# victordeleau/MUI-DeepAutoEncoder

Hardware: AMD Instinct MI355X
Metric: training samples/sec at 3x512-dim input, batch 8192 (higher is better)
Workload: dtype bf16; 1 GPU; embedding.yaml topology: 3 slots x 512 (io 1536), z=io, 4+4 layers -> 10 x Linear(1536,1536); batch 8192 rows per GPU, Adam lr 1e-5 wd 1e-4 clip 1.0, slot-blanking k=1; global_batch=8192, parallelism=dp1

## Files before the change

### include/codae_hip.h

```cpp
#ifndef CODAE_HIP_H
#define CODAE_HIP_H

#include <stddef.h>
#include <stdint.h>

#ifdef __cplusplus
extern "C" {
#endif

#define CODAE_ABI_VERSION 11

enum {
    CODAE_OK = 0,
    CODAE_E_INVALID = -1,
    CODAE_E_HIP = -2,
    CODAE_E_UNSUPPORTED = -3
};

enum {
    CODAE_PREC_F32 = 0,
    CODAE_PREC_BF16 = 1
};

enum {
// ... 181 lines not shown
int codae_side_stream(codae_handle h, void** stream_out);
int codae_join(codae_handle h, void* stream);

int codae_span_sumsq(const float* g, int64_t n, double* acc, void* stream);
int codae_step_update_span(codae_handle h, const codae_buffers* bufs, const codae_hyper* hyper, int64_t lo, int64_t hi,
                           const double* total_sq, void* stream);
int codae_sync_transposed(codae_handle h, const codae_buffers* bufs, void* stream);
int codae_train_step(codae_handle h, const codae_buffers* bufs, const codae_batch* batch,
                     const codae_hyper* hyper, void* stream);
int codae_dp_unique_id(void* out, int32_t capacity);
int codae_dp_init(codae_handle h, const void* unique_id, int32_t rank, int32_t world);
int codae_dp_destroy(codae_handle h);
int codae_train_step_dp(codae_handle h, const codae_buffers* bufs, const codae_batch* batch, const codae_hyper* hyper,
                        int32_t n_buckets, const int32_t* bucket_lo, const int32_t* bucket_hi, void* stream);
int codae_step_path(codae_handle h, const codae_buffers* bufs, int32_t B);
int codae_set_input_noise(codae_handle h, const codae_noise* noise);
int codae_set_loss_emphasis(codae_handle h, const codae_emphasis* emphasis);
int codae_set_recon_loss(codae_handle h, const codae_recon_loss* loss);
int codae_set_hidden_dropout(codae_handle h, const codae_dropout* d);
int codae_set_slot_contrast(codae_handle h, const codae_slot_contrast* contrast);
int codae_set_optimizer(codae_handle h, const codae_optimizer* opt);
int codae_set_slot_presence(codae_handle h, const uint8_t* present, int64_t n_rows, int32_t n_slots);
int codae_set_dataset_image(codae_handle h, const float* data, const void* image_bf16, int64_t n_rows, int32_t io);
int codae_set_tied_weights(codae_handle h, int32_t on);
int codae_graph_captures(codae_handle h);
int codae_eval_step(codae_handle h, const codae_buffers* bufs, const codae_batch* batch, float* out_y,
                    void* stream);

enum {
    CODAE_K_GEMM_FWD = 0,
    CODAE_K_GEMM_DGRAD = 1,
    CODAE_K_GEMM_WGRAD = 2,
    CODAE_K_LOSS = 3,
    CODAE_K_GATHER = 4,
    CODAE_K_SUMSQ = 5,
    CODAE_K_ADAM = 6,
    CODAE_K_SLAB_REDUCE = 7,
    CODAE_K_CHAIN = 8,
    CODAE_K_BIAS_FINISH = 9,
    CODAE_K_DROPOUT = 10,
    CODAE_K_COUNT = 11
};
int codae_profile_begin(codae_handle h, uint32_t class_mask, int32_t max_records);
int codae_profile_stride(codae_handle h, int32_t every_n_steps);
int codae_profile_end(codae_handle h, int32_t* kinds, float* ms, int32_t capacity, int32_t* n_out);

// ... 118 lines not shown
```

### mui-deepautoencoder_amd/codae/hip/__init__.py

```python
import ctypes as C
import os

_HERE = os.path.dirname(os.path.abspath(__file__))
LIB_PATH = os.environ.get("CODAE_HIP_LIB") or os.path.join(_HERE, "libcodae_hip.so")

PREC_F32 = 0
PREC_BF16 = 1

ABI_VERSION = 11
S_SQ_FULL, S_SQ_PARTIAL, S_GRAD_SQ, S_LAST_LOSS, S_STEP_SQ, S_CLIP_COEF = 0, 1, 2, 3, 4, 5
S_GRAD_SQ_SLOTS, S_N_SLOTS, S_ADAM_STEP, S_COUNT = 8, 64, 72, 80
ACT_NONE, ACT_RELU, ACT_LEAKY, ACT_RELU6, ACT_ELU, ACT_SOFTPLUS, ACT_HARDSIGMOID = 0, 1, 2, 3, 4, 5, 6
NOISE_NONE, NOISE_GAUSSIAN, NOISE_MASKING, NOISE_SALT_PEPPER = 0, 1, 2, 3
LOSS_MSE, LOSS_L1, LOSS_SMOOTH_L1, LOSS_HUBER, LOSS_SLOT_COSINE = 0, 1, 2, 3, 4
OPT_ADAM, OPT_ADAMW, OPT_SGD = 0, 1, 2
SCHED_CONSTANT, SCHED_COSINE, SCHED_LINEAR, SCHED_STEP = 0, 1, 2, 3
KERNEL_CLASSES = ("gemm_fwd", "gemm_dgrad", "gemm_wgrad", "loss", "gather", "sumsq", "adam", "slab_reduce", "chain",
                  "bias_finish", "dropout")


class HipError(RuntimeError):
    pass


# ... 84 lines not shown
    "codae_step_update": (C.c_int, [_P, C.POINTER(Buffers), C.POINTER(Hyper), _P]),
    "codae_step_backward_async": (C.c_int, [_P, C.POINTER(Buffers), _I32, _I32, _I32, _P]),
    "codae_side_stream": (C.c_int, [_P, C.POINTER(C.c_void_p)]),
    "codae_profile_stride": (C.c_int, [_P, _I32]),
    "codae_join": (C.c_int, [_P, _P]),
    "codae_span_sumsq": (C.c_int, [_P, _I64, _P, _P]),
    "codae_step_update_span": (C.c_int, [_P, C.POINTER(Buffers), C.POINTER(Hyper), _I64, _I64, _P, _P]),
    "codae_sync_transposed": (C.c_int, [_P, C.POINTER(Buffers), _P]),
    "codae_train_step": (C.c_int, [_P, C.POINTER(Buffers), C.POINTER(Batch), C.POINTER(Hyper), _P]),
    "codae_train_step_graph": (C.c_int, [_P, C.POINTER(Buffers), C.POINTER(Batch), C.POINTER(Hyper), _P]),
    "codae_set_input_noise": (C.c_int, [_P, C.POINTER(Noise)]),
    "codae_set_loss_emphasis": (C.c_int, [_P, C.POINTER(Emphasis)]),
    "codae_set_recon_loss": (C.c_int, [_P, C.POINTER(ReconLoss)]),
    "codae_set_hidden_dropout": (C.c_int, [_P, C.POINTER(Dropout)]),
    "codae_set_slot_contrast": (C.c_int, [_P, C.POINTER(SlotContrast)]),
    "codae_set_optimizer": (C.c_int, [_P, C.POINTER(Optimizer)]),
    "codae_optimizer_update": (C.c_int, [_P, _P, _P, _P, _P, _I64, C.POINTER(Hyper), C.POINTER(Optimizer), _P, _P]),
    "codae_graph_captures": (C.c_int, [_P]),
    "codae_set_tied_weights": (C.c_int, [_P, _I32]),
    "codae_tie_fold": (C.c_int, [_P, C.POINTER(TiePair), _I32, _P]),
    "codae_tie_mirror": (C.c_int, [_P, _P, _P, C.POINTER(TiePair), _I32, _P]),
    "codae_set_slot_presence": (C.c_int, [_P, _P, _I64, _I32]),
    "codae_set_dataset_image": (C.c_int, [_P, _P, _P, _I64, _I32]),
    "codae_corrupt_batch_present": (C.c_int, [C.POINTER(Batch), C.POINTER(Noise), _I32, _P, _P, _I32, _I64, _P, _I32, _P]),
    "codae_mse_loss_present": (C.c_int, [C.POINTER(Batch), _P, _P, _I32, _I64, _F, _P, _P, _P, _I32, _P]),
    "codae_emph_loss_present": (C.c_int, [C.POINTER(Batch), C.POINTER(Noise), _I32, C.POINTER(Emphasis), _P, _P, _I32, _I64, _F, _P, _P,
                                          _P, _I32, _P]),
    "codae_recon_loss_fwd_bwd_present": (C.c_int, [C.POINTER(Batch), C.POINTER(Noise), _I32, C.POINTER(Emphasis), C.POINTER(ReconLoss), _P,
                                                   _P, _I32, _I64, _F, _P, _P, _P, _I32, _P]),
    "codae_slot_contrast_prepare_present": (C.c_int, [_P, _I32, C.POINTER(SlotContrast), _I32, _I32, _P, _I32, _P]),
    "codae_slot_contrast_fwd_bwd_present": (C.c_int, [C.POINTER(Batch), C.POINTER(Noise), _I32, C.POINTER(Emphasis),
                                                      C.POINTER(SlotContrast), _P, _P, _I32, _I64, _F, _P, _P, _P, _I32, _P]),
    "codae_slot_contrast_ws_bytes": (_I64, [_I32, _I32, _I32, _I32]),
    "codae_slot_contrast_prepare": (C.c_int, [_P, _I32, C.POINTER(SlotContrast), _I32, _I32, _P]),
    "codae_slot_contrast_fwd_bwd": (C.c_int, [C.POINTER(Batch), C.POINTER(Noise), _I32, C.POINTER(Emphasis), C.POINTER(SlotContrast), _P, _P,
                                              _I32, _I64, _F, _P, _P, _P]),
    "codae_slot_contrast_blocks": (C.c_int, [_I32]),
    "codae_dropout_fwd": (C.c_int, [_P, _I32, _I64, _I32, _I32, _P, _I32, _I32, _F, C.c_uint64, _P]),
    "codae_dropout_bwd": (C.c_int, [_P, _I32, _I64, _I32, _I32, _P, _I32, _I32, _F, C.c_uint64, _P, _P]),
    "codae_dropout_blocks": (C.c_int, [_I32]),
    "codae_emph_loss": (C.c_int, [C.POINTER(Batch), C.POINTER(Noise), _I32, C.POINTER(Emphasis), _P, _P, _I32, _I64, _F, _P, _P, _P]),
    "codae_emph_loss_blocks": (C.c_int, [_I32]),
    "codae_recon_loss_fwd_bwd": (C.c_int, [C.POINTER(Batch), C.POINTER(Noise), _I32, C.POINTER(Emphasis), C.POINTER(ReconLoss), _P, _P, _I32, _I64,
                                           _F, _P, _P, _P]),
    "codae_recon_loss_blocks": (C.c_int, [_I32]),
    "codae_corrupt_batch": (C.c_int, [C.POINTER(Batch), C.POINTER(Noise), _I32, _P, _P, _I32, _I64, _P]),
# ... 100 lines not shown
```

### mui-deepautoencoder_amd/codae/hip/engine.py

```python
import ctypes as C

import torch

from . import (PREC_BF16, PREC_F32, S_COUNT, S_GRAD_SQ, S_GRAD_SQ_SLOTS, S_LAST_LOSS, S_N_SLOTS, S_SQ_FULL, S_SQ_PARTIAL,
               Batch, Buffers, Dropout, Emphasis,
               HipError, Hyper, Sizes, Spec, TiePair, check, current_stream, lib, ptr)


def precision_code(precision):
    if precision in (PREC_F32, "f32", "fp32", "parity"):
        return PREC_F32
    if precision in (PREC_BF16, "bf16", "throughput"):
        return PREC_BF16
    raise ValueError("unknown precision %r (use 'f32' or 'bf16')" % (precision,))


def _tie_pair_array(pairs):
    arr = (TiePair * max(len(pairs), 1))()
    for i, (e, d, r, c) in enumerate(pairs):
        arr[i] = TiePair(int(e), int(d), int(r), int(c))
    return arr


def tie_fold(grads, pairs):
# ... 59 lines not shown
            if int(sz.n_scalars) != S_COUNT:
                raise HipError("library reports %d scalars, binding expects %d" % (int(sz.n_scalars), S_COUNT))
            self.scalars = torch.zeros(int(sz.n_scalars), dtype=torch.float64, device=device)
        self.bufs = Buffers(ptr(self._params), ptr(self.grads), ptr(self.adam_m), ptr(self.adam_v), ptr(self.shadow),
                            ptr(self.acts), ptr(self.dacts), ptr(self.slabs), ptr(self.scalars), ptr(self.shadow_t),
                            ptr(self.bias_parts))
        self.w_off, self.b_off = [], []
        for l in range(self.L):
            w, b, s = C.c_int64(), C.c_int64(), C.c_int64()
            check(self._lib.codae_param_offsets(self._h, l, C.byref(w), C.byref(b), C.byref(s)))
            self.w_off.append(w.value)
            self.b_off.append(b.value)
        self.input_noise = None
        self.loss_emphasis = None
        self._emph_weights = None
        self.hidden_dropout = None
        self.recon_loss = None
        self.slot_contrast = None
        self._contrast_pins = None
        self.slot_presence = None
        self._presence_table = None
        self.tied_weights = False
        self._dataset_image = None
        self.optimizer = None
        self.adam_vmax = None
        self.step_count = 0
        self.generation = 0

    def _layer_acts(self, activation):
        if activation is None:
            return None
        if isinstance(activation, (list, tuple)) and len(activation) == self.L and all(
                isinstance(a, (list, tuple)) for a in activation):
            acts = [tuple(a) for a in activation]
        else:
            if isinstance(activation, (list, tuple)):
                one = tuple(activation)
            else:
                from ..model.activation import from_factory
                one = from_factory(activation)
            acts = [one if s[2] else (0, 0.0, 0.0, 0.0) for s in self.schedule]
        for a in acts:
            if len(a) != 4:
                raise HipError("activation per layer must be (kind, p0, p1, p2), got %r" % (a,))
        return [(int(a[0]), float(a[1]), float(a[2]), float(a[3])) for a in acts]

# ... 62 lines not shown
            check(self._lib.codae_backward(self._h, C.byref(self.bufs), ptr(dy), ptr(dx), dy.shape[0], layer_lo,
                                           layer_hi, current_stream()))
        return dx

    def make_batch(self, data, row_idx, mask_id, mask_table, B=None, mask_to_use=None, run=0):
        if data.dtype != torch.float32 or not data.is_contiguous() or data.device != self.device:
            raise HipError("batch data must be a contiguous fp32 tensor on %s" % self.device)
        for name, t in (("row_idx", row_idx), ("mask_id", mask_id)):
            if t is not None and (t.dtype != torch.int32 or t.device != self.device or not t.is_contiguous()):
                raise HipError("%s must be a contiguous int32 tensor on %s" % (name, self.device))
        if mask_table is not None and (mask_table.dtype != torch.uint8 or mask_table.device != self.device):
            raise HipError("mask_table must be a uint8 tensor on %s" % self.device)
        if B is None:
            B = int(row_idx.numel()) if row_idx is not None else int(data.shape[0])
        nb_run = 0
        if mask_to_use is not None:
            if mask_to_use.dtype != torch.int32 or mask_to_use.device != self.device or not mask_to_use.is_contiguous() \
                    or mask_to_use.dim() != 2 or mask_to_use.shape[0] != data.shape[0]:
                raise HipError("mask_to_use must be a contiguous int32 [n_rows, nb_run] tensor on %s" % self.device)
            nb_run = int(mask_to_use.shape[1])
        b = Batch(ptr(data), ptr(row_idx), ptr(mask_id), ptr(mask_table), int(B), int(data.shape[1]),
                  ptr(mask_to_use), nb_run, int(run))
        b._pinned = (data, row_idx, mask_id, mask_table, mask_to_use)
        return b

    def hyper(self, lr, weight_decay, clip=1.0, global_rows=0, betas=(0.9, 0.999), eps=1e-8, step=None):
        return Hyper(lr, weight_decay, betas[0], betas[1], eps, clip if clip else 0.0,
                     self.step_count + 1 if step is None else step, float(global_rows))

    def set_input_noise(self, noise):
        if noise is not None and not hasattr(noise, "as_struct"):
            raise HipError("set_input_noise: expected a codae.tool.InputNoise or None, got %r" % (noise,))
        st = None if noise is None else noise.as_struct()
        check(self._lib.codae_set_input_noise(self._h, None if st is None else C.byref(st)))
        self.input_noise = noise

    def set_loss_emphasis(self, emphasis, n_slots=None):
        if emphasis is not None and not hasattr(emphasis, "column_weights"):
            raise HipError("set_loss_emphasis: expected a codae.tool.LossEmphasis or None, got %r" % (emphasis,))
        weights = None
        if emphasis is not None:
            cw = emphasis.column_weights(self.schedule[-1][1], n_slots)
            if cw is not None:
                weights = torch.from_numpy(cw).to(self.device).contiguous()
        self._set_emphasis_struct(None if emphasis is None else Emphasis(emphasis.alpha, emphasis.beta, ptr(weights)))
        self._emph_weights = weights
# ... 235 lines not shown
```

### mui-deepautoencoder_amd/csrc/codae_common.h

```cpp
#pragma once
#include <hip/hip_runtime.h>
#include <stdint.h>
#include <stdio.h>
#include <type_traits>

#include "codae_hip.h"

namespace codae {

void set_error(const char* fmt, ...);

#define CODAE_HIP_CHECK(expr)                                                              \
    do {                                                                                   \
        hipError_t e_ = (expr);                                                            \
        if (e_ != hipSuccess) {                                                            \
            codae::set_error("%s failed: %s (%s:%d)", #expr, hipGetErrorString(e_), __FILE__, __LINE__); \
            return CODAE_E_HIP;                                                            \
        }                                                                                  \
    } while (0)

#define CODAE_LAUNCH_CHECK()                                                               \
    do {                                                                                   \
        hipError_t e_ = hipGetLastError();                                                 \
        if (e_ != hipSuccess) {                                                            \
// ... 169 lines not shown
    __device__ __forceinline__ void store16(void* p, uint32_t byte_off, u32x4 v) const {
        if constexpr (POL == STORE_PLAIN) *reinterpret_cast<u32x4*>(p) = v;
        else __builtin_amdgcn_raw_buffer_store_b128(v, rsrc, (int)byte_off, 0, 16);
    }
};

struct EnvToggles {
    int gemm_tile = -1;
    int gemm_dbg = 0;
    int wgrad_splitk = 0;
    int small_tile_max = 200;
    int small_stages = 4;
    int f32_gemm = 0;
    int group_tile = -1;
    bool side_priority_set = false; int side_priority = 0;
    bool no_wt = false, single_stream = false, tail_on_side = false, no_fused_loss = false, flat_adam = false,
         no_fused_norm = false, no_chain = false, no_deep_small = false,
         no_relu_bits = false,
         no_prefetch = false,
         no_defer_wgrad = false;
    bool no_folded_loss_finish = false;
    bool no_folded_bias_finish = false;
    bool no_dataset_image = false;
    int store_policy = -1;
};
const EnvToggles& env();
void env_reload();

struct GemmF32 {
    const float* A; int64_t a_rs, a_ks;
    const float* B; int64_t b_rs, b_ks;
    float* C; int64_t ldc;
    int M, N, K;
    const float* bias;
    int relu;
    const float* relu_src;
    int64_t ld_relu;
    float* colsum_part;
    const int* m_dev;
    int split_k;
    int act;
    float act_p[3];
};
int gemm_f32(const GemmF32& g, hipStream_t s);
int gemm_f32x3(const GemmF32& g, hipStream_t s);
bool gemm_f32x3_takes(const GemmF32& g);
// ... 1 lines not shown

constexpr int CODAE_GROUP_MAX = 16;
struct GemmF32Group {
    int n;
    GemmF32 g[CODAE_GROUP_MAX];
    int wg_begin[CODAE_GROUP_MAX + 1];
};
int gemm_f32x3_grouped(GemmF32Group& grp, hipStream_t s);

enum { OP_KC = 0,
       OP_KS = 1
};
struct LossFuse {
    int enabled;
    const float* data;
    const int32_t* row_idx;
    const int32_t* mask_id;
    const int32_t* mask_to_use;
    int nb_run, run;
    const uint8_t* table;
    int io;
    int B;
    float inv_n;
    double* parts;
};

struct GemmBf16 {
    const bf16_t* A; int64_t lda; int a_mode;
    const bf16_t* B; int64_t ldb; int b_mode;
    void* C; int64_t ldc; int c_f32;
    int M, N, K;
    const float* bias;
    int relu;
    const bf16_t* relu_src; int64_t ld_relu;
    float* colsum_part;
    int split_k;
    LossFuse loss;
    int dbg;
    uint8_t* relu_bits_out; const uint8_t* relu_bits; int64_t ld_bits;
    const void* prefetch; int64_t prefetch_bytes;
    int coscheduled;
    double* sumsq_slots;
    int act;
    float act_p[3];
    int store_policy;
};
// ... 156 lines not shown
```

### mui-deepautoencoder_amd/csrc/engine.hip

```cpp
#include <stdarg.h>
#include <stdlib.h>
#include <string.h>

#include <cmath>
#include <vector>

#include "layer_gemm.h"
#include <dlfcn.h>
#include <rccl/rccl.h>

namespace codae {

static thread_local char g_err[512] = "";

void set_error(const char* fmt, ...) {
    va_list ap;
    va_start(ap, fmt);
    vsnprintf(g_err, sizeof(g_err), fmt, ap);
    va_end(ap);
}

static EnvToggles g_env;
static bool g_env_loaded = false;

void env_reload() {
    EnvToggles e;
    if (const char* t = getenv("CODAE_GEMM_TILE")) {
        switch (t[0]) { case 's': e.gemm_tile = 0; break; case 'q': e.gemm_tile = 3; break; case 'x': e.gemm_tile = 6; break; case 'm': e.gemm_tile = 7; break; default: break; }
    }
    if (const char* d = getenv("CODAE_GEMM_DBG")) e.gemm_dbg = atoi(d);
    if (const char* k = getenv("CODAE_WGRAD_SPLITK")) e.wgrad_splitk = atoi(k) > 0 ? atoi(k) : 0;
    if (const char* k = getenv("CODAE_GROUP_TILE")) e.group_tile = (k[0] >= '0' && k[0] <= '2') ? k[0] - '0' : -1;
    if (const char* pr = getenv("CODAE_SIDE_PRIORITY")) { e.side_priority_set = true; e.side_priority = atoi(pr); }
    e.no_wt = getenv("CODAE_NO_WT") != nullptr;
    e.single_stream = getenv("CODAE_SINGLE_STREAM") != nullptr;
    e.tail_on_side = getenv("CODAE_TAIL_ON_SIDE") != nullptr;
    e.no_fused_loss = getenv("CODAE_NO_FUSED_LOSS") != nullptr;
    e.flat_adam = getenv("CODAE_FLAT_ADAM") != nullptr;
    e.no_fused_norm = getenv("CODAE_NO_FUSED_NORM") != nullptr;
    e.no_chain = getenv("CODAE_NO_CHAIN") != nullptr;
    e.no_deep_small = getenv("CODAE_NO_DEEP_SMALL") != nullptr;
    e.no_defer_wgrad = getenv("CODAE_NO_DEFER_WGRAD") != nullptr;
    e.no_prefetch = getenv("CODAE_NO_PREFETCH") != nullptr;
    e.no_relu_bits = getenv("CODAE_NO_RELU_BITS") != nullptr;
    e.no_folded_loss_finish = getenv("CODAE_NO_FOLDED_LOSS_FINISH") != nullptr;
    e.no_dataset_image = getenv("CODAE_NO_DATASET_IMAGE") != nullptr;
    e.no_folded_bias_finish = getenv("CODAE_NO_FOLDED_BIAS_FINISH") != nullptr;
    if (const char* k = getenv("CODAE_STORE_POLICY"))
        e.store_policy = !strcmp(k, "plain") ? STORE_PLAIN : (!strcmp(k, "wt") ? STORE_WT : -1);
    if (const char* k = getenv("CODAE_F32_GEMM")) e.f32_gemm = k[0] == 'n' ? 1 : (k[0] == 'x' ? 2 : 0);
    if (const char* k = getenv("CODAE_SMALL_TILE_MAX")) e.small_tile_max = atoi(k);
    if (const char* k = getenv("CODAE_SMALL_STAGES")) e.small_stages = atoi(k) == 2 ? 2 : 4;
    g_env = e;
    g_env_loaded = true;
}

const EnvToggles& env() {
    if (!g_env_loaded) env_reload();
    return g_env;
}

}

using namespace codae;

constexpr int CODAE_MAX_DACT = 16;

struct codae_engine {
    int L = 0;
    std::vector<int> in, out;
    std::vector<int> in_ld, out_ld;
    std::vector<uint8_t> relu;
    std::vector<uint8_t> act;
    std::vector<float> act_p;
    int max_batch = 0, max_rows = 0;
    int prec = CODAE_PREC_F32;
    std::vector<int64_t> w_off, b_off;
    int64_t n_param = 0, bias_begin = 0;
    int maxw = 0;
    std::vector<int64_t> act_off;
    int64_t act_bytes = 0, dact_one = 0, slab_bytes = 0;
    std::vector<int64_t> bits_off;
    int n_dact = 3;
    std::vector<int> split_k;
    std::vector<int64_t> part_off;
    int64_t part_floats = 0;
    int64_t loss_part_off = 0;
    int loss_part_cap = 0;
    bool chain_ok = false;
    struct PresCfg { const uint8_t* table; int64_t n_rows; int32_t n_slots; int32_t reserved; };
    struct DropCfg { float p[64]; uint64_t seed; int32_t on; int32_t reserved; };
    struct ImageCfg { const float* data; const void* image; int64_t n_rows; int32_t io; int32_t reserved; };
    struct TrainCfg {
        codae_noise noise;
        codae_emphasis emph;
        int32_t emph_on, reserved;
        codae_recon_loss recon;
        codae_slot_contrast contrast;
        PresCfg pres;
        DropCfg drop;
        codae_optimizer opt;
        int32_t tied, tied_reserved;
        ImageCfg img;
    } tc;
    bool recon_on() const { return tc.recon.kind != CODAE_LOSS_MSE; }
    bool contrast_on() const { return tc.contrast.weight != 0.f; }
    int n_free() const { return (L + 1) / 2; }
    std::vector<codae_tie_pair> tie_pairs;
    bool plain_mse() const { return !tc.emph_on && !recon_on() && !contrast_on() && tc.pres.table == nullptr; }
    int graph_captures = 0;
    bool drop_live = false;
    int drop_B = 0;
    const int32_t* drop_rows = nullptr;
    int32_t drop_step = 0;
    std::vector<int> parts_pending;
    hipStream_t side = nullptr;
    hipEvent_t ev_ready[CODAE_MAX_DACT] = {}, ev_join = nullptr, ev_w[CODAE_MAX_DACT] = {};
    unsigned ready_turn = 0;
    bool w_pending[CODAE_MAX_DACT] = {};
    bool side_dirty = false;
    bool norm_scalars_zero = false;
    bool prof_on = false;
    uint32_t prof_mask = 0;
    int prof_n = 0;
    int prof_every = 1, prof_step = 0;
    hipGraphExec_t graph_exec = nullptr;
// ... 985 lines not shown
        if (!noised && gathers_from_image(h, batch, act_ptr(h, b, 0)))
            rc = launch_gather_image(batch, reinterpret_cast<const bf16_t*>(h->tc.img.image), reinterpret_cast<bf16_t*>(act_ptr(h, b, 0)), s,
                                     h->in_ld[0], zero_norm, pres, pres_slots);
        else
            rc = launch_gather_noise(batch, noised ? &h->tc.noise : nullptr, noised ? hyper->step : 0, step_dev(h, b),
                                     act_ptr(h, b, 0), bf, s, h->in_ld[0], nullptr, zero_norm, pres, pres_slots);
    }
    if (rc) return rc;
    rc = zero_pad_rows(h, act_ptr(h, b, 0), B, rows, h->in_ld[0], s);
    if (rc) return rc;
    float* y = out_y ? out_y : reinterpret_cast<float*>(act_ptr(h, b, L));
    GroupScope fwd_group(h, CODAE_K_GEMM_FWD, s);
    if (h->drop_live) fwd_group.close();
    for (int l = 0; l < L; ++l) {
        const bool last = (l == L - 1);
        if (last && fuse_loss) {
            fwd_group.close();
            GemmBf16 g = layer_fwd_bf16(h, b, l, act_ptr(h, b, l), dact_ptr(h, b, l), h->out_ld[l], false, rows);
            g.colsum_part = part_ptr(h, b, l);
            g.loss.enabled = 1; g.loss.data = batch->data; g.loss.row_idx = batch->row_idx; g.loss.mask_id = batch->mask_id;
            g.loss.mask_to_use = batch->mask_to_use; g.loss.nb_run = batch->nb_run; g.loss.run = batch->run;
            g.loss.table = batch->mask_table; g.loss.io = batch->io; g.loss.B = B; g.loss.inv_n = (float)loss_inv_n(hyper, batch);
            g.loss.parts = loss_parts_ptr(h, b);
            if (b->shadow_wt != nullptr && l >= 1 && !h->cfg.no_wt && !h->cfg.no_prefetch) {
                g.prefetch = reinterpret_cast<const bf16_t*>(b->shadow_wt) + h->w_off[l];
                g.prefetch_bytes = (int64_t)h->in[l] * h->out[l] * 2;
            }
            const int n_loss_parts = gemm_bf16_loss_parts(g);
            CODAE_REQUIRE(n_loss_parts <= h->loss_part_cap, "fused loss: %d workgroups exceed the partial-sum rows (%d)", n_loss_parts, h->loss_part_cap);
            {
                ProfScope prof(h, CODAE_K_LOSS, s);
                rc = gemm_bf16(g, s);
            }
            if (rc) return rc;
            h->parts_pending[l] = gemm_bf16_colsum_rows(g);
            h->norm_scalars_zero = true;
            if (fold_finish) {
                fold->scalars = b->scalars; fold->inv_n = 1.0 / ((double)B * batch->io);
                fold->parts = loss_parts_ptr(h, b); fold->n_parts = n_loss_parts;
                return CODAE_OK;
            }
            return finish_loss(h, b, batch, n_loss_parts, s);
        }
        rc = last ? run_linear(h, b, l, act_ptr(h, b, l), y, true, B, s)
                  : run_linear(h, b, l, act_ptr(h, b, l), act_ptr(h, b, l + 1), false, rows, s);
        if (rc) return rc;
// ... 92 lines not shown
        CODAE_REQUIRE(n_rows >= 1, "codae_set_slot_presence: n_rows %lld must be >= 1", (long long)n_rows);
        CODAE_REQUIRE(!(h->recon_on() && h->tc.recon.kind == CODAE_LOSS_SLOT_COSINE) || h->tc.recon.n_slots == n_slots,
                      "codae_set_slot_presence: n_slots %d differs from slot_cosine's %d", n_slots, h->tc.recon.n_slots);
        CODAE_REQUIRE(!h->contrast_on() || (h->tc.contrast.n_slots == n_slots && (int64_t)h->tc.contrast.n_rows <= n_rows),
                      "codae_set_slot_presence: %d slots / %lld rows do not fit the slot contrast (%d slots, %d rows)", n_slots,
                      (long long)n_rows, h->tc.contrast.n_slots, h->tc.contrast.n_rows);
        p.table = present; p.n_rows = n_rows; p.n_slots = n_slots;
    }
    h->tc.pres = p;
    return CODAE_OK;
}

int codae_set_dataset_image(codae_handle h, const float* data, const void* image_bf16, int64_t n_rows, int32_t io) {
    CODAE_REQUIRE(h != nullptr, "codae_set_dataset_image: null handle");
    codae_engine::ImageCfg im{};
    if (image_bf16 != nullptr) {
        CODAE_REQUIRE(data != nullptr, "codae_set_dataset_image: an image without the dataset it was cast from");
        CODAE_REQUIRE(n_rows >= 1, "codae_set_dataset_image: n_rows %lld must be >= 1", (long long)n_rows);
        CODAE_REQUIRE(io == h->in[0], "codae_set_dataset_image: io %d does not match the model (%d)", io, h->in[0]);
        CODAE_REQUIRE((reinterpret_cast<uintptr_t>(image_bf16) & 15) == 0, "codae_set_dataset_image: the image must be 16-byte aligned");
        im.data = data; im.image = image_bf16; im.n_rows = n_rows; im.io = io;
    }
    h->tc.img = im;
    return CODAE_OK;
}

int codae_set_optimizer(codae_handle h, const codae_optimizer* opt) {
    CODAE_REQUIRE(h != nullptr, "codae_set_optimizer: null handle");
    int rc = check_optimizer(opt);
    if (rc) return rc;
    h->tc.opt = optimizer_canonical(opt);
    return CODAE_OK;
}

int codae_set_tied_weights(codae_handle h, int32_t on) {
    CODAE_REQUIRE(h != nullptr, "codae_set_tied_weights: null handle");
    if (on) {
        for (int l = 0; l < h->L / 2; ++l) {
            const int m = h->L - 1 - l;
            if (h->in[l] != h->out[m] || h->out[l] != h->in[m]) {
                set_error("tied weights: layers %d and %d are not mirror images (%d -> %d against %d -> %d)", l, m, h->in[l], h->out[l],
                          h->in[m], h->out[m]);
                return CODAE_E_UNSUPPORTED;
            }
        }
        h->tie_pairs.clear();
// ... 358 lines not shown
```

### mui-deepautoencoder_amd/csrc/gemm_bf16_pipe.hip

```cpp
#include "codae_common.h"
#include <type_traits>

namespace codae {
namespace {

#include "gemm_bf16_halftile.h"

constexpr int TIMELINE_WGS = 4096, TIMELINE_SLOTS = 6;
__device__ unsigned long long g_timeline[TIMELINE_WGS * TIMELINE_SLOTS];

constexpr int PARK_BIAS_BYTES = 1024;
template <int BM, int BN, bool C_F32, int EPI>
constexpr int pipe_smem_bytes() {
    const bool park = BM == 256;
    return 2 * (BM + BN) * 128 + (EPI == 3 ? BM * 8 : 0) + (park ? PARK_BIAS_BYTES : 0) + (park && !C_F32 && (EPI == 0 || EPI == 2 || EPI == 4) ? BM * BN / 8 : 0);
}

template <int BM, int BN, int WM, int WN, int NLB, int A_MODE, int B_MODE, bool C_F32, int DBG = 0, int EPI = 0, int POL = STORE_PLAIN>
__device__ __forceinline__ void gemm_bf16_pipe_tile(const GemmBf16& g, int tiles_n, int tiles_mn, int kt_total, int wg, int nwg,
                                                    char* smem_raw) {
    constexpr int NW = WM * WN;
    constexpr int SM = BM / WM, SN = BN / WN;
    constexpr int AHR = BM / 2, BHR = BN / 2;
    constexpr int TMH = SM / 32, TNH = SN / 32;
    constexpr int AH = AHR * 128, BH = BHR * 128;
    constexpr int BUF = 2 * AH + 2 * BH;
    constexpr int NLA = (NLB == 4 && NW == 8) ? 4 : (((AHR / 8) % NW == 0) ? NW : 8);
    constexpr int NA = AHR / 8 / NLA, NB = BHR / 8 / NLB;
    static_assert(NLB <= NW && NLA <= NW && (AHR / 8) % NLA == 0 && (BHR / 8) % NLB == 0, "loader waves");
    static_assert(SM % 32 == 0 && SN % 32 == 0, "wave sub-tile must split into 16-wide half tiles");
    lds_char* smem = (lds_char*)smem_raw;
    constexpr bool PARK = BM == 256;
    constexpr bool PARK_BITS = PARK && !C_F32 && (EPI == 0 || EPI == 2 || EPI == 4);
    constexpr int BIAS_OFF = 2 * BUF + (EPI == 3 ? BM * 8 : 0), BITS_OFF = BIAS_OFF + PARK_BIAS_BYTES;
    static_assert(BN * 4 <= PARK_BIAS_BYTES && BN % 32 == 0, "bias slice: one 16-B piece per lane of one wave");

    const int lane = threadIdx.x & 63;
    const int w = __builtin_amdgcn_readfirstlane(threadIdx.x >> 6);
    const int wr = w / WN, wc = w % WN;

    int bid = wg;
    if (nwg > 0) {
        const int q = nwg >> 3, r = nwg & 7, xcd = bid & 7;
        bid = (xcd < r ? xcd * (q + 1) : r * (q + 1) + (xcd - r) * q) + (bid >> 3);
    }
    const int z = bid / tiles_mn;
    const int tmn = bid - z * tiles_mn;
    constexpr int TILE_GROUP_M = 4;
    const int tiles_m = tiles_mn / tiles_n;
    const int grp = tmn / (TILE_GROUP_M * tiles_n);
    const int tm0 = grp * TILE_GROUP_M;
    const int gsz = tiles_m - tm0 < TILE_GROUP_M ? tiles_m - tm0 : TILE_GROUP_M;
    const int within = tmn - grp * (TILE_GROUP_M * tiles_n);
    const int tn = within / gsz, tm = tm0 + (within - tn * gsz);
    const int i0 = tm * BM, j0 = tn * BN;
    const int kt_begin = (int)((int64_t)kt_total * z / g.split_k);
    const int kt_end = (int)((int64_t)kt_total * (z + 1) / g.split_k);
// ... 17 lines not shown
        }
    }
    if constexpr (EPI == 3) {
        const LossFuse& L = g.loss;
        int* rowinfo = reinterpret_cast<int*>(smem_raw + 2 * BUF);
        for (int r = threadIdx.x; r < BM; r += 64 * NW) {
            const int i = i0 + r;
            int src = -1, id = 0;
            if (i < L.B && i < g.M) {
                src = L.row_idx ? L.row_idx[i] : i;
                if (L.mask_id != nullptr) id = L.mask_id[i];
                else if (L.mask_to_use != nullptr) id = L.mask_to_use[(int64_t)src * L.nb_run + L.run];
            }
            rowinfo[2 * r] = src; rowinfo[2 * r + 1] = id;
        }
    }

    const bool has_bias = g.bias != nullptr;
    if constexpr (PARK) {
        if (has_bias && w == NW - 1) {
            int j = j0 + 4 * lane;
            j = j + 4 <= g.N ? j : g.N - 4;
            __builtin_amdgcn_global_load_lds((gvoid*)(g.bias + j), (__attribute__((address_space(3))) void*)(smem + BIAS_OFF), 16, 0, 0);
        }
    }
    if constexpr (PARK_BITS) {
        if (g.relu_bits != nullptr) {
            constexpr int DPR = BN / 32, NI = BM * DPR / 64;
            static_assert((BM * DPR) % 64 == 0, "bit tile: whole 64-lane instructions");
#pragma unroll
            for (int q0 = 0; q0 < NI; q0 += NW) {
                const int ins = q0 + w;
                if (ins < NI) {
                    const int q = ins * 64 + lane, r = q / DPR, cd = q - r * DPR;
                    const int row = i0 + r < g.M ? i0 + r : g.M - 1;
                    int off = (j0 >> 3) + 4 * cd;
                    off = off + 4 <= (int)g.ld_bits ? off : (int)g.ld_bits - 4;
                    __builtin_amdgcn_global_load_lds((gvoid*)(g.relu_bits + (int64_t)row * g.ld_bits + off),
                                                     (__attribute__((address_space(3))) void*)(smem + BITS_OFF + ins * 256), 4, 0, 0);
                }
            }
        }
    }
    auto bias4 = [&](int jl) -> float4 {
        if constexpr (PARK) {
            const f32x4 v = *reinterpret_cast<const __attribute__((address_space(3))) f32x4*>(smem + BIAS_OFF + jl * 4);
// ... 191 lines not shown
        }
        asm volatile("" ::"v"(pf_val));
    };
    phase_barrier();
    if constexpr (EPI == 3) {
        const LossFuse& L = g.loss;
        const int* rowinfo = reinterpret_cast<const int*>(smem_raw + 2 * BUF);
        const bool masked = (L.mask_id != nullptr) || (L.mask_to_use != nullptr);
        const uint8_t* tb = masked ? L.table : reinterpret_cast<const uint8_t*>(L.data);
        constexpr int NT = 64 * NW;
        constexpr int PITCH = BN * 2 + 16;
        static_assert(BM * PITCH <= 2 * BUF, "output tile must fit in the staging buffers");
        float sq = 0.f, sqp = 0.f;
        float cs[2][TNH][4];
        int jcl[2][TNH];
        bool jok[2][TNH];
#pragma unroll
        for (int nh = 0; nh < 2; ++nh)
#pragma unroll
            for (int nt = 0; nt < TNH; ++nt) {
                const int j = j0 + nh * BHR + wc * (SN / 2) + 16 * nt + g4;
                jok[nh][nt] = j < g.N;
                jcl[nh][nt] = jok[nh][nt] ? j : 0;
                const float4 bj = bias4(nh * BHR + wc * (SN / 2) + 16 * nt + g4);
#pragma unroll
                for (int mh = 0; mh < 2; ++mh)
#pragma unroll
                    for (int mt = 0; mt < TMH; ++mt) {
                        acc[mh][mt][nh][nt][0] += bj.x; acc[mh][mt][nh][nt][1] += bj.y;
                        acc[mh][mt][nh][nt][2] += bj.z; acc[mh][mt][nh][nt][3] += bj.w;
                    }
#pragma unroll
                for (int k = 0; k < 4; ++k) cs[nh][nt][k] = 0.f;
            }
        const int jbase = j0 + wc * (SN / 2) + g4;
        auto loss_rows = [&](auto full_tag) {
            constexpr bool FULL = decltype(full_tag)::value;
#pragma unroll
            for (int mh = 0; mh < 2; ++mh) {
                float4 xv[TMH][2][TNH];
                uint32_t mk[TMH][2][TNH];
                bool live[TMH];
#pragma unroll
                for (int mt = 0; mt < TMH; ++mt) {
                    const int il = mh * AHR + wr * (SM / 2) + 16 * mt + li;
                    const int src = rowinfo[2 * il], id = rowinfo[2 * il + 1];
                    live[mt] = src >= 0;
                    const float* xrow = L.data + (int64_t)(src >= 0 ? src : 0) * L.io;
                    const uint8_t* mrow = tb + (int64_t)id * L.io;
#pragma unroll
                    for (int nh = 0; nh < 2; ++nh)
#pragma unroll
                        for (int nt = 0; nt < TNH; ++nt) {
                            const int off = FULL ? jbase + (nh * BHR + 16 * nt) : jcl[nh][nt];
                            xv[mt][nh][nt] = *reinterpret_cast<const float4*>(xrow + off);
                            const uint32_t mv = *reinterpret_cast<const uint32_t*>(mrow + off);
                            mk[mt][nh][nt] = masked ? mv : 0x01010101u;
                        }
                }
#pragma unroll
                for (int mt = 0; mt < TMH; ++mt) {
                    const int il = mh * AHR + wr * (SM / 2) + 16 * mt + li;
#pragma unroll
                    for (int nh = 0; nh < 2; ++nh)
#pragma unroll
                        for (int nt = 0; nt < TNH; ++nt) {
                            const int jl = nh * BHR + wc * (SN / 2) + 16 * nt + g4;
                            const f32x4 a = acc[mh][mt][nh][nt];
                            const float4 x = xv[mt][nh][nt];
                            const float yv[4] = {a[0], a[1], a[2], a[3]};
                            const float xs[4] = {x.x, x.y, x.z, x.w};
                            const bool on = live[mt] && (FULL || jok[nh][nt]);
                            float gq[4];
#pragma unroll
                            for (int k = 0; k < 4; ++k) {
                                const float d = on ? xs[k] - yv[k] : 0.f;
                                const float se = d * d;
                                sq += se;
                                asm volatile("" : "+v"(sq));
                                sqp += ((mk[mt][nh][nt] >> (8 * k)) & 0xffu) == 0 ? se : 0.f;
                                gq[k] = on ? -2.f * d * L.inv_n : 0.f;
                                cs[nh][nt][k] += gq[k];
                            }
                            u32x2 o;
                            o[0] = pack_bf16x2(gq[0], gq[1]);
                            o[1] = pack_bf16x2(gq[2], gq[3]);
                            *reinterpret_cast<__attribute__((address_space(3))) u32x2*>(smem + il * PITCH + jl * 2) = o;
                        }
                }
                __builtin_amdgcn_sched_barrier(0);
            }
        };
        if (j0 + BN <= g.N) loss_rows(std::true_type{}); else loss_rows(std::false_type{});
        stamp(3);
        phase_barrier();
        {
            constexpr int CH = BN / 8, RL = NT / CH;
            const int c = threadIdx.x % CH, rl = threadIdx.x / CH;
            const int j = j0 + c * 8;
            bf16_t* Cb = reinterpret_cast<bf16_t*>(g.C);
            const TileStore<POL> out(Cb + (int64_t)i0 * g.ldc);
            constexpr int ITER = (BM + RL - 1) / RL;
#pragma unroll
            for (int it = 0; it < ITER; ++it) {
                const int r = rl + it * RL;
                const bool ok = rl < RL && j < g.N && r < BM && i0 + r < g.M;
                const u32x4 lv = *reinterpret_cast<const __attribute__((address_space(3))) u32x4*>(smem + (ok ? r : 0) * PITCH + c * 16);
                if (ok) out.store16(Cb + (int64_t)(i0 + r) * g.ldc + j, (uint32_t)(r * (int)g.ldc + j) * 2u, lv);
            }
        }
        if constexpr (dbg_time) { wait_vmcnt<0>(); stamp(4); }
#pragma unroll
        for (int o2 = 32; o2 > 0; o2 >>= 1) { sq += __shfl_xor(sq, o2); sqp += __shfl_xor(sqp, o2); }
#pragma unroll
        for (int nh = 0; nh < 2; ++nh)
#pragma unroll
            for (int nt = 0; nt < TNH; ++nt)
#pragma unroll
                for (int k = 0; k < 4; ++k) {
                    float v = cs[nh][nt][k];
                    v += __shfl_xor(v, 1); v += __shfl_xor(v, 2); v += __shfl_xor(v, 4); v += __shfl_xor(v, 8);
                    cs[nh][nt][k] = v;
                }
        phase_barrier();
        float* red = reinterpret_cast<float*>(smem_raw);
        static_assert((WM * BN + 2 * NW) * 4 <= 2 * BUF, "reduction scratch must fit");
        if (li == 0) {
#pragma unroll
            for (int nh = 0; nh < 2; ++nh)
#pragma unroll
                for (int nt = 0; nt < TNH; ++nt) {
                    const int jl = nh * BHR + wc * (SN / 2) + 16 * nt + g4;
#pragma unroll
// ... 454 lines not shown
```

Baseline: 7.333 million samples/s.

## Park the slot mask table in LDS and pipeline loss-epilogue row fetches

The Python engine now registers the batch mask table with the native handle. When the table has at most 16 masks, the fused loss GEMM epilogue copies each tile's mask slices into shared memory with global_load_lds instead of reading a mask row from global memory per output row. With the masks parked, the epilogue also double-buffers its work by quarters: it fetches the data rows for the next quarter while computing the current one, hiding load latency. The cost is extra LDS per block, which may lower occupancy, plus more register pressure. Partial tiles fall back to the old path.

```diff
diff --git a/include/codae_hip.h b/include/codae_hip.h
--- a/include/codae_hip.h
+++ b/include/codae_hip.h
@@ -227,6 +227,7 @@
 int codae_set_optimizer(codae_handle h, const codae_optimizer* opt);
 int codae_set_slot_presence(codae_handle h, const uint8_t* present, int64_t n_rows, int32_t n_slots);
 int codae_set_dataset_image(codae_handle h, const float* data, const void* image_bf16, int64_t n_rows, int32_t io);
+int codae_set_mask_table(codae_handle h, const uint8_t* mask_table, int32_t n_masks);
 int codae_set_tied_weights(codae_handle h, int32_t on);
 int codae_graph_captures(codae_handle h);
 int codae_eval_step(codae_handle h, const codae_buffers* bufs, const codae_batch* batch, float* out_y,
diff --git a/mui-deepautoencoder_amd/codae/hip/__init__.py b/mui-deepautoencoder_amd/codae/hip/__init__.py
--- a/mui-deepautoencoder_amd/codae/hip/__init__.py
+++ b/mui-deepautoencoder_amd/codae/hip/__init__.py
@@ -130,6 +130,7 @@
     "codae_tie_mirror": (C.c_int, [_P, _P, _P, C.POINTER(TiePair), _I32, _P]),
     "codae_set_slot_presence": (C.c_int, [_P, _P, _I64, _I32]),
     "codae_set_dataset_image": (C.c_int, [_P, _P, _P, _I64, _I32]),
+    "codae_set_mask_table": (C.c_int, [_P, _P, _I32]),
     "codae_corrupt_batch_present": (C.c_int, [C.POINTER(Batch), C.POINTER(Noise), _I32, _P, _P, _I32, _I64, _P, _I32, _P]),
     "codae_mse_loss_present": (C.c_int, [C.POINTER(Batch), _P, _P, _I32, _I64, _F, _P, _P, _P, _I32, _P]),
     "codae_emph_loss_present": (C.c_int, [C.POINTER(Batch), C.POINTER(Noise), _I32, C.POINTER(Emphasis), _P, _P, _I32, _I64, _F, _P, _P,
diff --git a/mui-deepautoencoder_amd/codae/hip/engine.py b/mui-deepautoencoder_amd/codae/hip/engine.py
--- a/mui-deepautoencoder_amd/codae/hip/engine.py
+++ b/mui-deepautoencoder_amd/codae/hip/engine.py
@@ -105,6 +105,7 @@
         self._presence_table = None
         self.tied_weights = False
         self._dataset_image = None
+        self._mask_table_known = None
         self.optimizer = None
         self.adam_vmax = None
         self.step_count = 0
@@ -213,6 +214,12 @@
         b = Batch(ptr(data), ptr(row_idx), ptr(mask_id), ptr(mask_table), int(B), int(data.shape[1]),
                   ptr(mask_to_use), nb_run, int(run))
         b._pinned = (data, row_idx, mask_id, mask_table, mask_to_use)
+        known = None
+        if mask_table is not None and mask_table.dim() == 2 and mask_table.is_contiguous() and mask_table.shape[1] == data.shape[1]:
+            known = (ptr(mask_table), int(mask_table.shape[0]))
+        if known != self._mask_table_known:
+            check(self._lib.codae_set_mask_table(self._h, *(known or (None, 0))))
+            self._mask_table_known = known
         return b
 
     def hyper(self, lr, weight_decay, clip=1.0, global_rows=0, betas=(0.9, 0.999), eps=1e-8, step=None):
diff --git a/mui-deepautoencoder_amd/csrc/codae_common.h b/mui-deepautoencoder_amd/csrc/codae_common.h
--- a/mui-deepautoencoder_amd/csrc/codae_common.h
+++ b/mui-deepautoencoder_amd/csrc/codae_common.h
@@ -215,6 +215,7 @@
     bool no_folded_loss_finish = false;
     bool no_folded_bias_finish = false;
     bool no_dataset_image = false;
+    bool no_loss_mask_park = false;
     int store_policy = -1;
 };
 const EnvToggles& env();
@@ -262,6 +263,7 @@
     int io;
     int B;
     float inv_n;
+    int n_masks;
     double* parts;
 };
 
diff --git a/mui-deepautoencoder_amd/csrc/engine.hip b/mui-deepautoencoder_amd/csrc/engine.hip
--- a/mui-deepautoencoder_amd/csrc/engine.hip
+++ b/mui-deepautoencoder_amd/csrc/engine.hip
@@ -46,6 +46,7 @@
     e.no_folded_loss_finish = getenv("CODAE_NO_FOLDED_LOSS_FINISH") != nullptr;
     e.no_dataset_image = getenv("CODAE_NO_DATASET_IMAGE") != nullptr;
     e.no_folded_bias_finish = getenv("CODAE_NO_FOLDED_BIAS_FINISH") != nullptr;
+    e.no_loss_mask_park = getenv("CODAE_NO_LOSS_MASK_PARK") != nullptr;
     if (const char* k = getenv("CODAE_STORE_POLICY"))
         e.store_policy = !strcmp(k, "plain") ? STORE_PLAIN : (!strcmp(k, "wt") ? STORE_WT : -1);
     if (const char* k = getenv("CODAE_F32_GEMM")) e.f32_gemm = k[0] == 'n' ? 1 : (k[0] == 'x' ? 2 : 0);
@@ -91,6 +92,7 @@
     struct PresCfg { const uint8_t* table; int64_t n_rows; int32_t n_slots; int32_t reserved; };
     struct DropCfg { float p[64]; uint64_t seed; int32_t on; int32_t reserved; };
     struct ImageCfg { const float* data; const void* image; int64_t n_rows; int32_t io; int32_t reserved; };
+    struct MaskCfg { const uint8_t* table; int32_t n_masks; int32_t reserved; };
     struct TrainCfg {
         codae_noise noise;
         codae_emphasis emph;
@@ -102,6 +104,7 @@
         codae_optimizer opt;
         int32_t tied, tied_reserved;
         ImageCfg img;
+        MaskCfg masks;
     } tc;
     bool recon_on() const { return tc.recon.kind != CODAE_LOSS_MSE; }
     bool contrast_on() const { return tc.contrast.weight != 0.f; }
@@ -1133,6 +1136,7 @@
             g.loss.mask_to_use = batch->mask_to_use; g.loss.nb_run = batch->nb_run; g.loss.run = batch->run;
             g.loss.table = batch->mask_table; g.loss.io = batch->io; g.loss.B = B; g.loss.inv_n = (float)loss_inv_n(hyper, batch);
             g.loss.parts = loss_parts_ptr(h, b);
+            if (!h->cfg.no_loss_mask_park && batch->mask_table != nullptr && batch->mask_table == h->tc.masks.table) g.loss.n_masks = h->tc.masks.n_masks;
             if (b->shadow_wt != nullptr && l >= 1 && !h->cfg.no_wt && !h->cfg.no_prefetch) {
                 g.prefetch = reinterpret_cast<const bf16_t*>(b->shadow_wt) + h->w_off[l];
                 g.prefetch_bytes = (int64_t)h->in[l] * h->out[l] * 2;
@@ -1271,6 +1275,17 @@
         im.data = data; im.image = image_bf16; im.n_rows = n_rows; im.io = io;
     }
     h->tc.img = im;
+    return CODAE_OK;
+}
+
+int codae_set_mask_table(codae_handle h, const uint8_t* mask_table, int32_t n_masks) {
+    CODAE_REQUIRE(h != nullptr, "codae_set_mask_table: null handle");
+    codae_engine::MaskCfg m{};
+    if (mask_table != nullptr) {
+        CODAE_REQUIRE(n_masks >= 1, "codae_set_mask_table: n_masks %d must be >= 1", n_masks);
+        m.table = mask_table; m.n_masks = n_masks;
+    }
+    h->tc.masks = m;
     return CODAE_OK;
 }
 
diff --git a/mui-deepautoencoder_amd/csrc/gemm_bf16_pipe.hip b/mui-deepautoencoder_amd/csrc/gemm_bf16_pipe.hip
--- a/mui-deepautoencoder_amd/csrc/gemm_bf16_pipe.hip
+++ b/mui-deepautoencoder_amd/csrc/gemm_bf16_pipe.hip
@@ -10,10 +10,12 @@
 __device__ unsigned long long g_timeline[TIMELINE_WGS * TIMELINE_SLOTS];
 
 constexpr int PARK_BIAS_BYTES = 1024;
+constexpr int PARK_MASKS = 16;
 template <int BM, int BN, bool C_F32, int EPI>
 constexpr int pipe_smem_bytes() {
     const bool park = BM == 256;
-    return 2 * (BM + BN) * 128 + (EPI == 3 ? BM * 8 : 0) + (park ? PARK_BIAS_BYTES : 0) + (park && !C_F32 && (EPI == 0 || EPI == 2 || EPI == 4) ? BM * BN / 8 : 0);
+    return 2 * (BM + BN) * 128 + (EPI == 3 ? BM * 8 : 0) + (park ? PARK_BIAS_BYTES : 0) + (park && EPI == 3 ? PARK_MASKS * BN : 0) +
+           (park && !C_F32 && (EPI == 0 || EPI == 2 || EPI == 4) ? BM * BN / 8 : 0);
 }
 
 template <int BM, int BN, int WM, int WN, int NLB, int A_MODE, int B_MODE, bool C_F32, int DBG = 0, int EPI = 0, int POL = STORE_PLAIN>
@@ -33,6 +35,7 @@
     constexpr bool PARK = BM == 256;
     constexpr bool PARK_BITS = PARK && !C_F32 && (EPI == 0 || EPI == 2 || EPI == 4);
     constexpr int BIAS_OFF = 2 * BUF + (EPI == 3 ? BM * 8 : 0), BITS_OFF = BIAS_OFF + PARK_BIAS_BYTES;
+    constexpr int MASK_OFF = BIAS_OFF + PARK_BIAS_BYTES;
     static_assert(BN * 4 <= PARK_BIAS_BYTES && BN % 32 == 0, "bias slice: one 16-B piece per lane of one wave");
 
     const int lane = threadIdx.x & 63;
@@ -96,6 +99,30 @@
             int j = j0 + 4 * lane;
             j = j + 4 <= g.N ? j : g.N - 4;
             __builtin_amdgcn_global_load_lds((gvoid*)(g.bias + j), (__attribute__((address_space(3))) void*)(smem + BIAS_OFF), 16, 0, 0);
+        }
+    }
+    bool mask_parked = false;
+    if constexpr (EPI == 3 && PARK) {
+        const LossFuse& L = g.loss;
+        mask_parked = (L.mask_id != nullptr || L.mask_to_use != nullptr) && L.n_masks >= 1 && L.n_masks <= PARK_MASKS;
+        if (mask_parked) {
+            constexpr int PPR = BN / 4, NI_MAX = PARK_MASKS * PPR / 64;
+            static_assert((PARK_MASKS * PPR) % 64 == 0, "mask slices: whole 64-lane instructions");
+            const int ni = (L.n_masks * PPR + 63) >> 6;
+#pragma unroll
+            for (int q0 = 0; q0 < NI_MAX; q0 += NW) {
+                const int ins = q0 + (NW - 1 - w);
+                if (ins < ni) {
+                    const int q = ins * 64 + lane;
+                    int m = q / PPR;
+                    const int cg = q - m * PPR;
+                    m = m < L.n_masks ? m : L.n_masks - 1;
+                    int j = j0 + 4 * cg;
+                    j = j + 4 <= g.N ? j : g.N - 4;
+                    __builtin_amdgcn_global_load_lds((gvoid*)(L.table + (int64_t)m * L.io + j),
+                                                     (__attribute__((address_space(3))) void*)(smem + MASK_OFF + ins * 256), 4, 0, 0);
+                }
+            }
         }
     }
     if constexpr (PARK_BITS) {
@@ -333,6 +360,12 @@
                 const int j = j0 + nh * BHR + wc * (SN / 2) + 16 * nt + g4;
                 jok[nh][nt] = j < g.N;
                 jcl[nh][nt] = jok[nh][nt] ? j : 0;
+            }
+        const int jbase = j0 + wc * (SN / 2) + g4;
+#pragma unroll
+        for (int nh = 0; nh < 2; ++nh)
+#pragma unroll
+            for (int nt = 0; nt < TNH; ++nt) {
                 const float4 bj = bias4(nh * BHR + wc * (SN / 2) + 16 * nt + g4);
 #pragma unroll
                 for (int mh = 0; mh < 2; ++mh)
@@ -344,82 +377,107 @@
 #pragma unroll
                 for (int k = 0; k < 4; ++k) cs[nh][nt][k] = 0.f;
             }
-        const int jbase = j0 + wc * (SN / 2) + g4;
-        auto loss_rows = [&](auto full_tag) {
-            constexpr bool FULL = decltype(full_tag)::value;
-#pragma unroll
-            for (int mh = 0; mh < 2; ++mh) {
-                float4 xv[TMH][2][TNH];
-                uint32_t mk[TMH][2][TNH];
-                bool live[TMH];
-#pragma unroll
-                for (int mt = 0; mt < TMH; ++mt) {
-                    const int il = mh * AHR + wr * (SM / 2) + 16 * mt + li;
-                    const int src = rowinfo[2 * il], id = rowinfo[2 * il + 1];
-                    live[mt] = src >= 0;
-                    const float* xrow = L.data + (int64_t)(src >= 0 ? src : 0) * L.io;
-                    const uint8_t* mrow = tb + (int64_t)id * L.io;
-#pragma unroll
-                    for (int nh = 0; nh < 2; ++nh)
-#pragma unroll
-                        for (int nt = 0; nt < TNH; ++nt) {
-                            const int off = FULL ? jbase + (nh * BHR + 16 * nt) : jcl[nh][nt];
-                            xv[mt][nh][nt] = *reinterpret_cast<const float4*>(xrow + off);
+        auto write_dy = [&]() {
+            stamp(3);
+            phase_barrier();
+            {
+                constexpr int CH = BN / 8, RL = NT / CH;
+                const int c = threadIdx.x % CH, rl = threadIdx.x / CH;
+                const int j = j0 + c * 8;
+                bf16_t* Cb = reinterpret_cast<bf16_t*>(g.C);
+                const TileStore<POL> out(Cb + (int64_t)i0 * g.ldc);
+                constexpr int ITER = (BM + RL - 1) / RL;
+    #pragma unroll
+                for (int it = 0; it < ITER; ++it) {
+                    const int r = rl + it * RL;
+                    const bool ok = rl < RL && j < g.N && r < BM && i0 + r < g.M;
+                    const u32x4 lv = *reinterpret_cast<const __attribute__((address_space(3))) u32x4*>(smem + (ok ? r : 0) * PITCH + c * 16);
+                    if (ok) out.store16(Cb + (int64_t)(i0 + r) * g.ldc + j, (uint32_t)(r * (int)g.ldc + j) * 2u, lv);
+                }
+            }
+        };
+        auto loss_rows = [&](auto full_tag, auto park_tag) {
+            constexpr bool FULL = decltype(full_tag)::value, MPARK = decltype(park_tag)::value;
+            constexpr int NQ = 2 * TMH;
+            static_assert(TMH >= 2, "two quarters in flight");
+            float4 xv[TMH][2][TNH];
+            uint32_t mk[TMH][2][TNH];
+            bool live[TMH];
+            auto fetch = [&](int q) {
+                const int mh = q / TMH, mt = q % TMH, s = mt;
+                const int il = mh * AHR + wr * (SM / 2) + 16 * mt + li;
+                const int src = rowinfo[2 * il], id = rowinfo[2 * il + 1];
+                live[s] = src >= 0;
+                const float* xrow = L.data + (int64_t)(src >= 0 ? src : 0) * L.io;
+                const uint8_t* mrow = tb + (int64_t)id * L.io;
+#pragma unroll
+                for (int nh = 0; nh < 2; ++nh)
+#pragma unroll
+                    for (int nt = 0; nt < TNH; ++nt) {
+                        const int off = FULL ? jbase + (nh * BHR + 16 * nt) : jcl[nh][nt];
+                        xv[s][nh][nt] = *reinterpret_cast<const float4*>(xrow + off);
+                        if constexpr (MPARK) {
+                            const int jl = nh * BHR + wc * (SN / 2) + 16 * nt + g4;
+                            mk[s][nh][nt] = *reinterpret_cast<const __attribute__((address_space(3))) uint32_t*>(smem + MASK_OFF + id * BN + jl);
+                        } else {
                             const uint32_t mv = *reinterpret_cast<const uint32_t*>(mrow + off);
-                            mk[mt][nh][nt] = masked ? mv : 0x01010101u;
+                            mk[s][nh][nt] = masked ? mv : 0x01010101u;
                         }
-                }
-#pragma unroll
-                for (int mt = 0; mt < TMH; ++mt) {
-                    const int il = mh * AHR + wr * (SM / 2) + 16 * mt + li;
-#pragma unroll
-                    for (int nh = 0; nh < 2; ++nh)
-#pragma unroll
-                        for (int nt = 0; nt < TNH; ++nt) {
-                            const int jl = nh * BHR + wc * (SN / 2) + 16 * nt + g4;
-                            const f32x4 a = acc[mh][mt][nh][nt];
-                            const float4 x = xv[mt][nh][nt];
-                            const float yv[4] = {a[0], a[1], a[2], a[3]};
-                            const float xs[4] = {x.x, x.y, x.z, x.w};
-                            const bool on = live[mt] && (FULL || jok[nh][nt]);
-                            float gq[4];
-#pragma unroll
-                            for (int k = 0; k < 4; ++k) {
-                                const float d = on ? xs[k] - yv[k] : 0.f;
-                                const float se = d * d;
-                                sq += se;
-                                asm volatile("" : "+v"(sq));
-                                sqp += ((mk[mt][nh][nt] >> (8 * k)) & 0xffu) == 0 ? se : 0.f;
-                                gq[k] = on ? -2.f * d * L.inv_n : 0.f;
-                                cs[nh][nt][k] += gq[k];
-                            }
-                            u32x2 o;
-                            o[0] = pack_bf16x2(gq[0], gq[1]);
-                            o[1] = pack_bf16x2(gq[2], gq[3]);
-                            *reinterpret_cast<__attribute__((address_space(3))) u32x2*>(smem + il * PITCH + jl * 2) = o;
+                    }
+            };
+            auto compute = [&](int q) {
+                const int mh = q / TMH, mt = q % TMH, s = mt;
+                const int il = mh * AHR + wr * (SM / 2) + 16 * mt + li;
+#pragma unroll
+                for (int nh = 0; nh < 2; ++nh)
+#pragma unroll
+                    for (int nt = 0; nt < TNH; ++nt) {
+                        const int jl = nh * BHR + wc * (SN / 2) + 16 * nt + g4;
+                        const f32x4 a = acc[mh][mt][nh][nt];
+                        const float4 x = xv[s][nh][nt];
+                        const float yv[4] = {a[0], a[1], a[2], a[3]};
+                        const float xs[4] = {x.x, x.y, x.z, x.w};
+                        const bool on = live[s] && (FULL || jok[nh][nt]);
+                        float gq[4];
+#pragma unroll
+                        for (int k = 0; k < 4; ++k) {
+                            const float d = on ? xs[k] - yv[k] : 0.f;
+                            const float se = d * d;
+                            sq += se;
+                            asm volatile("" : "+v"(sq));
+                            sqp += ((mk[s][nh][nt] >> (8 * k)) & 0xffu) == 0 ? se : 0.f;
+                            gq[k] = on ? -2.f * d * L.inv_n : 0.f;
+                            cs[nh][nt][k] += gq[k];
                         }
-                }
-                __builtin_amdgcn_sched_barrier(0);
+                        u32x2 o;
+                        o[0] = pack_bf16x2(gq[0], gq[1]);
+                        o[1] = pack_bf16x2(gq[2], gq[3]);
+                        *reinterpret_cast<__attribute__((address_space(3))) u32x2*>(smem + il * PITCH + jl * 2) = o;
+                    }
+            };
+            if constexpr (MPARK) {
+                fetch(0);
+#pragma unroll
+                for (int q = 0; q < NQ; ++q) {
+                    if (q + 1 < NQ) fetch(q + 1);
+                    compute(q);
+                    __builtin_amdgcn_sched_barrier(0);
+                }
+            } else {
+#pragma unroll
+                for (int mh = 0; mh < 2; ++mh) {
+#pragma unroll
+                    for (int mt = 0; mt < TMH; ++mt) fetch(mh * TMH + mt);
+#pragma unroll
+                    for (int mt = 0; mt < TMH; ++mt) compute(mh * TMH + mt);
+                    __builtin_amdgcn_sched_barrier(0);
+                }
             }
         };
-        if (j0 + BN <= g.N) loss_rows(std::true_type{}); else loss_rows(std::false_type{});
-        stamp(3);
-        phase_barrier();
-        {
-            constexpr int CH = BN / 8, RL = NT / CH;
-            const int c = threadIdx.x % CH, rl = threadIdx.x / CH;
-            const int j = j0 + c * 8;
-            bf16_t* Cb = reinterpret_cast<bf16_t*>(g.C);
-            const TileStore<POL> out(Cb + (int64_t)i0 * g.ldc);
-            constexpr int ITER = (BM + RL - 1) / RL;
-#pragma unroll
-            for (int it = 0; it < ITER; ++it) {
-                const int r = rl + it * RL;
-                const bool ok = rl < RL && j < g.N && r < BM && i0 + r < g.M;
-                const u32x4 lv = *reinterpret_cast<const __attribute__((address_space(3))) u32x4*>(smem + (ok ? r : 0) * PITCH + c * 16);
-                if (ok) out.store16(Cb + (int64_t)(i0 + r) * g.ldc + j, (uint32_t)(r * (int)g.ldc + j) * 2u, lv);
-            }
-        }
+        const bool full_tile = j0 + BN <= g.N;
+        if (mask_parked && full_tile) loss_rows(std::true_type{}, std::true_type{});
+        else loss_rows(std::false_type{}, std::false_type{});
+        write_dy();
         if constexpr (dbg_time) { wait_vmcnt<0>(); stamp(4); }
 #pragma unroll
         for (int o2 = 32; o2 > 0; o2 >>= 1) { sq += __shfl_xor(sq, o2); sqp += __shfl_xor(sqp, o2); }
```

Result: no change. 7.355 million samples/s, median of 6 (+0.3%).
